# view-sonic/Cloud-Server

Measured on AMD Instinct MI355X. Metric: train_samples_per_s, higher is better.
Workload: dtype fp32; 1 GPU; model=reference sample CNN (API.md:306-332), 2,276,218 params, global_batch=50, per_gpu_batch=50, optimizer=AdagradOptimizer, parallelism=dp1, backend=hip, hip_graph=True, collectives=none, xgmi=single rank

## Files before the change

cloud_server_amd/csrc/kernels/dense_update.h:

```cpp
#pragma once
#include "common.h"
#include "optim_common.h"

namespace csa {

typedef float du_f32x4 __attribute__((ext_vector_type(4)));
typedef unsigned int du_u32x4 __attribute__((ext_vector_type(4)));

constexpr int DU_FT = 16;
constexpr int DU_SUB = 2;
constexpr int DU_MAXM = 64;
constexpr int DU_KS = DU_MAXM / 4;
constexpr int MAXC_DU = 128;
constexpr int DU_SLAB = 16;
constexpr int DU_PART = DU_MAXM * DU_FT;
constexpr size_t DU_LDS_MAX = 150 * 1024;

struct DUArgs {
  int M, K, N;
  const float* dY;
  float* W;
  float* bias;
  float* dX;
  const float* x_fwd;
  int act; float alpha;
  BNRef bn; int bn_on;
  const float* bn_tab;
  float* bwd_slab;
  int det;
  const float* Xw;
  int opt; float lr; const int64_t* step;
  float* s0w; float* s1w;
  float* s0b; float* s1b;
  float scale;
  float* gW; float* gb;
  int cs;
  float* part;
  unsigned* cnt;
  const float* hy;
  const float* hdl;
  float* hgw; float* hgb;
  const float* hrl; const int* hrc;
  float* ring_loss; int* ring_correct; int ring; float ldiv;
  int hact; float halpha;
  float* hw; float* hb; float* hs0w; float* hs1w; float* hs0b; float* hs1b;
};

constexpr int DU_HNC = 10;

constexpr int DU_MAXDEF = 4;
struct DUDeferred {
  DUArgs seg[DU_MAXDEF];
  int blocks[DU_MAXDEF];
  int n = 0;
  int head = -1;
};
extern thread_local DUDeferred g_du_def;

struct DUSegs {
  DUArgs seg[DU_MAXDEF];
  int start[DU_MAXDEF + 1];
  int nseg, head;
};
int du_take(DUSegs& out);
int du_flush_segs(const DUSegs& u, hipStream_t st);
}
extern "C" int csa_dense_update_flush(hipStream_t st);
namespace csa {


static __constant__ long long* g_du_dbg = nullptr;
#define DU_STAMP(i)                                                                          \
  do {                                                                                       \
    if (g_du_dbg && threadIdx.x == 0) g_du_dbg[bid * 16 + (i)] = (long long)__builtin_amdgcn_s_memrealtime(); \
  } while (0)

__host__ __device__ constexpr int du_nb(int waves) { return 32 * waves; }
constexpr int DU_FOLD_FS = 5, DU_FOLD_BLK = DU_FT * DU_FOLD_FS;
__host__ __device__ constexpr int du_upo_hw_floats() { return 64 * (8 + 10); }
__host__ __device__ inline size_t du_upo_lds_floats(int M) {
  const size_t m4 = (size_t)((M + 3) & ~3);
  const size_t tail = 1024 > du_upo_hw_floats() ? 1024 : du_upo_hw_floats();
  return 2 * m4 * 64 + tail;
}
__host__ __device__ inline size_t du_lds_floats(int M, int waves) {
  const size_t a = (size_t)M * (du_nb(waves) + 4), b = (size_t)waves * 4 * 4 * DU_FOLD_BLK;
  return (a > b ? a : b) + DU_MAXM * DU_FT + 6 * MAXC_DU + 4;
}

__device__ __forceinline__ du_u32x4 du_bits(float4 v) { du_u32x4 u; __builtin_memcpy(&u, &v, 16); return u; }
__device__ __forceinline__ float4 du_f4(du_u32x4 u) { float4 v; __builtin_memcpy(&v, &u, 16); return v; }

template <int NSLOT>
__device__ __forceinline__ void du_store_w(const DUArgs& a, const float4 (&wv)[DU_SUB], const float4 (&s0v)[DU_SUB],
                                           const float4 (&s1v)[DU_SUB], const long (&wofs)[DU_SUB],
                                           const bool (&sok)[DU_SUB], int i, int nf, bool bown, int bn0, float bw,
                                           float bs0, float bs1) {
  if (bown && (threadIdx.x & 63) == 0) {
    (a.gW ? a.gb : a.bias)[bn0] = bw;
    if (NSLOT >= 1) a.s0b[bn0] = bs0;
    if (NSLOT >= 2) a.s1b[bn0] = bs1;
  }
#pragma unroll
  for (int j = 0; j < DU_SUB; ++j) {
    if (!sok[j] || i >= nf) continue;
    *reinterpret_cast<float4*>((a.gW ? a.gW : a.W) + wofs[j]) = wv[j];
    if (NSLOT >= 1) *reinterpret_cast<float4*>(a.s0w + wofs[j]) = s0v[j];
    if (NSLOT >= 2) *reinterpret_cast<float4*>(a.s1w + wofs[j]) = s1v[j];
  }
}

constexpr int DU_HMAXR = 8;

struct DUHead {
  int hn0, nh;
  float hy[2];
  float dl[3];
};

template <int THREADS>
__device__ __forceinline__ void du_head_prefetch(const DUArgs& a, int grp, int groups, int cb, int nb, DUHead& h) {
  const int hper = (nb + groups - 1) / groups;
  h.hn0 = cb + grp * hper;
  h.nh = max(0, min(hper, cb + nb - h.hn0));
  const int t = threadIdx.x;
#pragma unroll
  for (int u = 0; u < 2; ++u) {
    const int e = t + u * THREADS, m = e / DU_HMAXR, r = e % DU_HMAXR;
    h.hy[u] = a.hy[(long)min(m, a.M - 1) * a.N + min(h.hn0 + min(r, max(h.nh - 1, 0)), a.N - 1)];
  }
  const int n10 = a.M * DU_HNC;
#pragma unroll
  for (int u = 0; u < 3; ++u) h.dl[u] = a.hdl[min(t + u * THREADS, n10 - 1)];
}

template <int THREADS>
__device__ __forceinline__ void du_head_finish(const DUArgs& a, DUHead& h, float* s_hw, bool last_block) {
  const int t = threadIdx.x, M = a.M;
  float* s_y = s_hw;
  float* s_d = s_hw + 64 * DU_HMAXR;
  pin(h.hy[0]); pin(h.hy[1]); pin(h.dl[0]); pin(h.dl[1]); pin(h.dl[2]);
  if (t < M * DU_HMAXR) s_y[t] = act_fwd(h.hy[0], a.hact, a.halpha);
  if (t + THREADS < M * DU_HMAXR) s_y[t + THREADS] = act_fwd(h.hy[1], a.hact, a.halpha);
#pragma unroll
  for (int u = 0; u < 3; ++u)
    if (t + u * THREADS < M * DU_HNC) s_d[t + u * THREADS] = h.dl[u];
  __syncthreads();
  const int outs = h.nh * DU_HNC;
  for (int o = t; o < outs; o += THREADS) {
    const int rr = o / DU_HNC, j = o - rr * DU_HNC, n = h.hn0 + rr;
    float v = 0.f;
    if (h.nh <= DU_HMAXR) {
      for (int m = 0; m < M; ++m) v = fmaf(s_y[m * DU_HMAXR + rr], s_d[m * DU_HNC + j], v);
    } else {
      for (int m = 0; m < M; ++m) v = fmaf(act_fwd(a.hy[(long)m * a.N + n], a.hact, a.halpha), s_d[m * DU_HNC + j], v);
    }
    if (a.hw) {
      const long k = (long)n * DU_HNC + j;
      float w = a.hw[k], z0 = a.hs0w ? a.hs0w[k] : 0.f, z1 = a.hs1w ? a.hs1w[k] : 0.f;
      opt_update(a.opt, opt_step_lr(a.opt, a.lr, a.step), w, v, z0, z1);
      a.hw[k] = w;
      if (a.hs0w) a.hs0w[k] = z0;
      if (a.hs1w) a.hs1w[k] = z1;
    } else {
      a.hgw[(long)n * DU_HNC + j] = v;
    }
  }
  if (last_block) {
    const int lane = t & 63, w = t >> 6;
    if (w == 0) {
      if (lane < DU_HNC) {
        float v = 0.f;
        for (int m = 0; m < M; ++m) v += s_d[m * DU_HNC + lane];
        if (a.hb) {
          float wb = a.hb[lane], z0 = a.hs0b ? a.hs0b[lane] : 0.f, z1 = a.hs1b ? a.hs1b[lane] : 0.f;
          opt_update(a.opt, opt_step_lr(a.opt, a.lr, a.step), wb, v, z0, z1);
          a.hb[lane] = wb;
          if (a.hs0b) a.hs0b[lane] = z0;
          if (a.hs1b) a.hs1b[lane] = z1;
        } else {
          a.hgb[lane] = v;
        }
      }
    } else if (w == 1) {
      float l = lane < M ? a.hrl[lane] : 0.f;
      float c = lane < M ? (float)a.hrc[lane] : 0.f;
      l = wave_sum(l);
      c = wave_sum(c);
      if (lane == 0) {
        const int pos = (int)((*a.step - 1) % a.ring);
        a.ring_loss[pos] = l / a.ldiv;
        a.ring_correct[pos] = (int)(c + 0.5f);
      }
    }
  }
}

template <int NSLOT, int WAVES, bool HEAD, bool DGO = false, bool UPO = false>
__device__ __forceinline__ void du_body(const DUArgs& a, const int bid, const int nblk, float* smem) {
  constexpr int THREADS = 64 * WAVES, NB = du_nb(WAVES), SN = NB + 4, HW = 16 * WAVES;
  const int M = a.M, K = a.K, N = a.N, cs = a.cs;
  static_assert(!UPO || WAVES == 4, "the update-only body is the 4-wave carried form");
  float* sdy = smem;
  float* s_bn = smem + du_lds_floats(M, WAVES) - 6 * MAXC_DU - 4;
  const int M4 = (M + 3) & ~3;
  float* sxw = UPO ? smem + 2 * M4 * 64 : s_bn - DU_MAXM * DU_FT;
  float* s_st = s_bn + 4 * MAXC_DU;
  int* s_flag = reinterpret_cast<int*>(s_st + 2 * MAXC_DU);
  const int tid = threadIdx.x, lane = tid & 63;
  const int wave = __builtin_amdgcn_readfirstlane(tid >> 6);
  const int i = lane & 15, q = lane >> 4;
  const int grp = bid / cs, cblk = bid - grp * cs;
  const int f0 = grp * DU_FT, nf = min(DU_FT, K - f0);
  const int cb = cblk * NB, nb = min(NB, N - cb);
  const int groups = nblk / cs;
  const bool dgrad = !UPO && a.dX != nullptr;
  const bool tf = dgrad && (a.act != ACT_NONE || a.bn_on);
  const bool tabs = a.bn_on && a.bn_tab;
  const int C = a.bn.C > 0 ? a.bn.C : 1;
  constexpr int nslot = NSLOT;
  DU_STAMP(0);
  float* s_hw;
  if constexpr (UPO) {
    s_hw = sxw;
  } else {
    __shared__ float s_hw_st[HEAD ? 64 * (DU_HMAXR + DU_HNC) : 1];
    s_hw = s_hw_st;
  }
  DUHead hd;

  float xw1[1024 / THREADS];
#pragma unroll
  for (int u = 0; u < 1024 / THREADS; ++u) {
    const int e = u * THREADS + tid;
    if (!DGO) xw1[u] = a.Xw[(long)min(e >> 4, M - 1) * K + f0 + min(e & 15, nf - 1)];
  }
  const float* tsrc = tabs ? a.bn_tab : a.Xw;
  float tv[512 / THREADS > 0 ? 512 / THREADS : 1];
  constexpr int NTV = UPO ? 0 : (512 / THREADS > 0 ? 512 / THREADS : 1);
#pragma unroll
  for (int u = 0; u < NTV; ++u) {
    const int e = u * THREADS + tid;
    tv[u] = tsrc[tabs && e < 4 * C ? e : 0];
  }
  const int n4 = N >> 2;
  int h4[DU_SUB];
#pragma unroll
  for (int j = 0; j < DU_SUB; ++j) h4[j] = max(min(nb - HW * j, HW), 0) >> 2;
  const float* b0 = nslot >= 1 ? a.s0w : a.W;
  const float* b1 = nslot >= 2 ? a.s1w : a.W;
  const int frow = f0 + min(i, nf - 1);
  float4 dyv[DU_SUB][4], wv[DU_SUB], s0v[DU_SUB], s1v[DU_SUB];
  long wofs[DU_SUB];
  bool sok[DU_SUB];
#pragma unroll
  for (int j = 0; j < DU_SUB; ++j) {
    if constexpr (UPO) {
      const int nch = M4 >> 2;
#pragma unroll
      for (int u = 0; u < DU_MAXM / 16; ++u) {
        const int c = min(wave + 4 * u, nch - 1);
        const int r = 4 * c + (lane >> 4), cq = ((lane & 15) - r) & 15;
        const float* src = a.dY + (long)min(r, M - 1) * N + cb + HW * j + 4 * cq;
        __builtin_amdgcn_global_load_lds(src, sdy + (j * M4 + 4 * c) * 64, 16, 0, 0);
      }
    } else {
#pragma unroll
    for (int u = 0; u < 4; ++u) {
      const int e = u * THREADS + tid;
      int row = 0, c4 = 0;
      if (h4[j] == HW / 4) { row = e / (HW / 4); c4 = e % (HW / 4); }
      else if (h4[j] > 0) { row = e / h4[j]; c4 = e - row * h4[j]; }
      dyv[j][u] = reinterpret_cast<const float4*>(a.dY)[min(row, M - 1) * n4 + (h4[j] > 0 ? (cb + HW * j) / 4 + c4 : 0)];
    }
    }
    const int lc = 16 * (wave + WAVES * j);
    sok[j] = lc < nb;
    wofs[j] = (long)frow * N + cb + min(lc, nb - 16) + 4 * q;
    wv[j] = *reinterpret_cast<const float4*>(a.W + wofs[j]);
    s0v[j] = s1v[j] = make_float4(0.f, 0.f, 0.f, 0.f);
    if (nslot >= 1) s0v[j] = *reinterpret_cast<const float4*>(b0 + wofs[j]);
    if (nslot >= 2) s1v[j] = *reinterpret_cast<const float4*>(b1 + wofs[j]);
  }
  const int bper = (nb + groups - 1) / groups;
  const int bn0 = cb + grp * bper + wave;
  const bool bown = !DGO && (a.bias || a.gW) && wave < bper && grp * bper + wave < nb;
  const int bnc = bown ? bn0 : 0;
  float bw = (a.bias ? a.bias : a.dY)[bnc];
  float bs0 = (nslot >= 1 && a.bias ? a.s0b : a.dY)[bnc];
  float bs1 = (nslot >= 2 && a.bias ? a.s1b : a.dY)[bnc];
  const int em = tid >> 2, fq = 4 * (tid & 3);
  const bool eitem = tid < 256;
  const float* xsrc = tf && a.x_fwd ? a.x_fwd : a.Xw;
  float4 xf = make_float4(0.f, 0.f, 0.f, 0.f);
  if (!UPO) xf = *reinterpret_cast<const float4*>(xsrc + (long)min(em, M - 1) * K + f0 + min(fq, nf - 4));
  if (HEAD) du_head_prefetch<THREADS>(a, grp, groups, cb, nb, hd);

  const float lr = opt_step_lr(a.opt, a.lr, a.step);
  du_f32x4 dacc[4];
#pragma unroll
  for (int t = 0; t < 4; ++t) dacc[t] = du_f32x4{0.f, 0.f, 0.f, 0.f};
  float xb[DU_KS];
#pragma unroll
  for (int j = 0; j < DU_SUB; ++j) {
    if (j == 0) {
#pragma unroll
      for (int u = 0; u < 1024 / THREADS; ++u) {
        if (DGO) break;
        const int e = u * THREADS + tid;
        pin(xw1[u]);
        sxw[e] = ((e >> 4) < M && (e & 15) < nf) ? xw1[u] : 0.f;
      }
#pragma unroll
      for (int u = 0; u < NTV; ++u) {
        const int e = u * THREADS + tid;
        pin(tv[u]);
        if (tabs && e < 4 * C) s_bn[(e / C) * MAXC_DU + e % C] = tv[u];
      }
    }
    if constexpr (!UPO) {
#pragma unroll
    for (int u = 0; u < 4; ++u) pin(dyv[j][u]);
#pragma unroll
    for (int u = 0; u < 4; ++u) {
      const int e = u * THREADS + tid;
      if (h4[j] > 0 && e < M * h4[j]) {
        const int row = h4[j] == HW / 4 ? e / (HW / 4) : e / h4[j];
        const int c4 = e - row * h4[j];
        *reinterpret_cast<float4*>(sdy + row * SN + HW * j + 4 * c4) = dyv[j][u];
      }
    }
    }
    if (j == 0 && a.bn_on && dgrad && !tabs)
      bn_reduce_to_lds(a.bn, s_bn, s_bn + MAXC_DU, s_bn + 2 * MAXC_DU, s_bn + 3 * MAXC_DU, s_st);
    __syncthreads();
    if (UPO && j == 1) DU_STAMP(4);
    if (j == 0) {
      DU_STAMP(1);
#pragma unroll
      for (int s = 0; s < DU_KS; ++s) xb[s] = DGO ? 0.f : sxw[(4 * s + q) * DU_FT + i];
    }
    pin(wv[j]); pin(s0v[j]); pin(s1v[j]);
    if (j == 0) DU_STAMP(2);
    if (UPO && j == 1) DU_STAMP(5);
    if (!sok[j]) continue;
    const int n0 = 16 * (wave + WAVES * j);
    const float wk[4] = {wv[j].x, wv[j].y, wv[j].z, wv[j].w};
    if (dgrad) {
#pragma unroll
      for (int t = 0; t < 4; ++t) {
        if (16 * t >= M) break;
        const float4 d4 = *reinterpret_cast<const float4*>(sdy + min(16 * t + i, M - 1) * SN + n0 + 4 * q);
        const float ak[4] = {d4.x, d4.y, d4.z, d4.w};
#pragma unroll
        for (int k = 0; k < 4; ++k) dacc[t] = __builtin_amdgcn_mfma_f32_16x16x4f32(ak[k], i < nf ? wk[k] : 0.f, dacc[t], 0, 0, 0);
      }
    }
    if (DGO) continue;
    du_f32x4 g0 = du_f32x4{0.f, 0.f, 0.f, 0.f}, g1 = g0;
    const float* col = sdy + n0 + i;
    float av[DU_KS];
    if constexpr (UPO) {
      const float* hb = sdy + j * M4 * 64;
      const int lc = 16 * wave + i;
#pragma unroll
      for (int s = 0; s < DU_KS; ++s) {
        const int r = min(4 * s + q, M - 1);
        av[s] = hb[r * 64 + ((((lc >> 2) + r) & 15) << 2) + (lc & 3)];
      }
    } else {
#pragma unroll
      for (int s = 0; s < DU_KS; ++s) av[s] = col[min(4 * s + q, M - 1) * SN];
    }
#pragma unroll
    for (int s = 0; s < DU_KS; s += 2) {
      g0 = __builtin_amdgcn_mfma_f32_16x16x4f32(av[s], xb[s], g0, 0, 0, 0);
      g1 = __builtin_amdgcn_mfma_f32_16x16x4f32(av[s + 1], xb[s + 1], g1, 0, 0, 0);
    }
    float w[4] = {wv[j].x, wv[j].y, wv[j].z, wv[j].w};
    float s0[4] = {s0v[j].x, s0v[j].y, s0v[j].z, s0v[j].w};
    float s1[4] = {s1v[j].x, s1v[j].y, s1v[j].z, s1v[j].w};
#pragma unroll
    for (int r = 0; r < 4; ++r) {
      if (a.gW) w[r] = (g0[r] + g1[r]) * a.scale;
      else opt_update(a.opt, lr, w[r], (g0[r] + g1[r]) * a.scale, s0[r], s1[r]);
    }
    wv[j] = make_float4(w[0], w[1], w[2], w[3]);
    s0v[j] = make_float4(s0[0], s0[1], s0[2], s0[3]);
    s1v[j] = make_float4(s1[0], s1[1], s1[2], s1[3]);
    if (UPO && j == 0) DU_STAMP(7);
    if (UPO && j == 1) DU_STAMP(8);
  }
  pin(bw); pin(bs0); pin(bs1); pin(xf);
  if (bown) {
    for (int u = wave; u < bper; u += WAVES) {
      const int lcol = grp * bper + u;
      if (lcol >= nb) break;
      const int n = cb + lcol;
      float v;
      if constexpr (UPO) {
        const int lh = lcol & 63;
        v = lane < M ? sdy[((lcol >> 6) * M4 + lane) * 64 + ((((lh >> 2) + lane) & 15) << 2) + (lh & 3)] : 0.f;
      } else {
        v = lane < M ? sdy[lane * SN + lcol] : 0.f;
      }
      v = wave_sum(v);
      if (lane == 0) {
        if (u == wave) {
          if (a.gW) bw = v * a.scale;
          else opt_update(a.opt, lr, bw, v * a.scale, bs0, bs1);
        } else {
          float cw = 0.f, c0 = 0.f, c1 = 0.f;
          if (!a.gW) {
            cw = a.bias[n];
            if (nslot >= 1) c0 = a.s0b[n];
            if (nslot >= 2) c1 = a.s1b[n];
          }
          if (a.gW) cw = v * a.scale;
          else opt_update(a.opt, lr, cw, v * a.scale, c0, c1);
          (a.gW ? a.gb : a.bias)[n] = cw;
          if (nslot >= 1) a.s0b[n] = c0;
          if (nslot >= 2) a.s1b[n] = c1;
        }
      }
    }
  }
  DU_STAMP(3);
  if (HEAD) du_head_finish<THREADS>(a, hd, s_hw, bid == nblk - 1);
  if (!dgrad) {
    if (!DGO) du_store_w<NSLOT>(a, wv, s0v, s1v, wofs, sok, i, nf, bown, bn0, bw, bs0, bs1);
    DU_STAMP(6);
    return;
  }

  __syncthreads();
  float* fold = sdy;
#pragma unroll
  for (int t = 0; t < 4; ++t) {
    if (16 * t >= M) break;
    float* dst = fold + ((wave * 4 + t) * 4 + q) * DU_FOLD_BLK + DU_FOLD_FS * i;
#pragma unroll
    for (int r = 0; r < 4; ++r) dst[r] = dacc[t][r];
  }
  __syncthreads();
  DU_STAMP(4);
  float4 g4 = make_float4(0.f, 0.f, 0.f, 0.f);
  if (eitem && em < M) {
    const int t = em >> 4, qq = (em >> 2) & 3, r = em & 3;
    const float* src = fold + (t * 4 + qq) * DU_FOLD_BLK + DU_FOLD_FS * fq + r;
#pragma unroll
    for (int w = 0; w < WAVES; ++w) {
      const float* p = src + w * 4 * 4 * DU_FOLD_BLK;
      g4.x += p[0]; g4.y += p[DU_FOLD_FS]; g4.z += p[2 * DU_FOLD_FS]; g4.w += p[3 * DU_FOLD_FS];
    }
  }
  if (cs > 1) {
    const __amdgpu_buffer_rsrc_t prs = __builtin_amdgcn_make_buffer_rsrc(
        a.part, 0, (int)((size_t)nblk * DU_PART * sizeof(float)), 0x00020000);
    if (eitem && em < M)
      __builtin_amdgcn_raw_buffer_store_b128(du_bits(g4), prs, (int)(((size_t)bid * DU_PART + em * DU_FT + fq) * 4), 0, 16);
    asm volatile("s_waitcnt vmcnt(0)" ::: "memory");
    __syncthreads();
    if (tid == 0) {
      const unsigned old = __hip_atomic_fetch_add(a.cnt + grp, 1u, __ATOMIC_RELAXED, __HIP_MEMORY_SCOPE_AGENT);
      const int last = old == (unsigned)(cs - 1);
      if (last) __hip_atomic_store(a.cnt + grp, 0u, __ATOMIC_RELAXED, __HIP_MEMORY_SCOPE_AGENT);
      *s_flag = last;
    }
    __syncthreads();
    if (!DGO) du_store_w<NSLOT>(a, wv, s0v, s1v, wofs, sok, i, nf, bown, bn0, bw, bs0, bs1);
    if (!*s_flag) return;
    __builtin_amdgcn_fence(__ATOMIC_ACQUIRE, "wavefront");
    g4 = make_float4(0.f, 0.f, 0.f, 0.f);
    if (eitem && em < M) {
      float4 v[8];
      for (int c0 = 0; c0 < cs; c0 += 8) {
#pragma unroll
        for (int u = 0; u < 8; ++u)
          v[u] = du_f4(__builtin_amdgcn_raw_buffer_load_b128(
              prs, (int)((((size_t)grp * cs + min(c0 + u, cs - 1)) * DU_PART + em * DU_FT + fq) * 4), 0, 16));
#pragma unroll
        for (int u = 0; u < 8; ++u)
          if (c0 + u < cs) { g4.x += v[u].x; g4.y += v[u].y; g4.z += v[u].z; g4.w += v[u].w; }
      }
    }
  } else {
    if (!DGO) du_store_w<NSLOT>(a, wv, s0v, s1v, wofs, sok, i, nf, bown, bn0, bw, bs0, bs1);
  }
  float v1[4] = {0.f, 0.f, 0.f, 0.f}, v2[4] = {0.f, 0.f, 0.f, 0.f};
  if (eitem && em < M && fq < nf) {
    float g[4] = {g4.x, g4.y, g4.z, g4.w};
    const float x[4] = {xf.x, xf.y, xf.z, xf.w};
    if (tf) {
      int ch = (f0 + fq) % C;
#pragma unroll
      for (int r = 0; r < 4; ++r, ch = (ch + 1 == C) ? 0 : ch + 1) {
        const float z = a.bn_on ? x[r] * s_bn[2 * MAXC_DU + ch] + s_bn[3 * MAXC_DU + ch] : x[r];
        const float y = act_fwd(z, a.act, a.alpha);
        g[r] = act_bwd(g[r], z, y, a.act, a.alpha);
        v1[r] = g[r];
        v2[r] = a.bn_on ? g[r] * (x[r] - s_bn[ch]) * s_bn[MAXC_DU + ch] : 0.f;
      }
    }
    out_store4(a.dX + (long)em * K + f0 + fq, make_float4(g[0], g[1], g[2], g[3]));
  }
  DU_STAMP(5);
  if (a.bn_on && a.bwd_slab) {
#pragma unroll
    for (int r = 0; r < 4; ++r) {
#pragma unroll
      for (int o = 4; o < 64; o <<= 1) {
        v1[r] += __shfl_xor(v1[r], o, 64);
        v2[r] += __shfl_xor(v2[r], o, 64);
      }
    }
    float* sred = sxw;
    if (eitem && lane < 4) {
#pragma unroll
      for (int r = 0; r < 4; ++r) {
        sred[wave * 32 + 4 * lane + r] = v1[r];
        sred[wave * 32 + 16 + 4 * lane + r] = v2[r];
      }
    }
    __syncthreads();
    if (a.det) {
      if (tid < 2 * C) {
        const int st = tid / C, c = tid - st * C;
        float acc = 0.f;
        for (int ff = 0; ff < nf; ++ff)
          if ((f0 + ff) % C == c) {
            const int e = 16 * st + ff;
            acc += sred[e] + sred[32 + e] + sred[64 + e] + sred[96 + e];
          }
        a.bwd_slab[(size_t)grp * 2 * C + tid] = acc;
      }
    } else if (tid < 32 && (tid & 15) < nf) {
      const float acc = sred[tid] + sred[32 + tid] + sred[64 + tid] + sred[96 + tid];
      const int st = tid >> 4, c = (f0 + (tid & 15)) % C;
      atomicAdd(a.bwd_slab + (size_t)(grp % DU_SLAB) * 2 * C + st * C + c, acc);
    }
  }
  DU_STAMP(6);
}

template <int NSLOT, bool HEADOK>
__device__ __forceinline__ void du_segs_body(const DUSegs& u, int e, float* smem) {
  int s = 0;
#pragma unroll
  for (int k = 1; k < DU_MAXDEF; ++k) s += (k < u.nseg && e >= u.start[k]) ? 1 : 0;
  const DUArgs& d = u.seg[s];
  const int lb = e - u.start[s], nb = u.start[s + 1] - u.start[s];
  if (HEADOK && s == u.head) du_body<NSLOT, 4, true, false, true>(d, lb, nb, smem);
  else du_body<NSLOT, 4, false, false, true>(d, lb, nb, smem);
}

}
```

cloud_server_amd/csrc/kernels/dense_update.hip:

```cpp
#include "dense_update.h"
#include <cstdlib>

namespace csa {

template <int NSLOT, int WAVES, bool HEAD, bool DGO = false>
__global__ __launch_bounds__(64 * WAVES) void dense_bwd_update_kernel(DUArgs a) {
  extern __shared__ __attribute__((aligned(16))) float smem[];
  du_body<NSLOT, WAVES, HEAD, DGO>(a, (int)blockIdx.x, (int)gridDim.x, smem);
}

thread_local DUDeferred g_du_def{};

}


using namespace csa;

static thread_local float* g_du_grad_w = nullptr;
static thread_local float* g_du_grad_b = nullptr;

CSA_NT_SETTER(csa_nt_out_du)

CSA_API int csa_du_debug(long long* p) {
  return (int)hipMemcpyToSymbol(HIP_SYMBOL(g_du_dbg), &p, sizeof(p));
}

CSA_API int csa_dense_bwd_update_ok(int M, int K, int N, int bn_C) {
  if (M < 1 || M > DU_MAXM || K < 4 || K % 4 || N < 16 || N % 16) return 0;
  if (bn_C > MAXC_DU) return 0;
  if (N > 512 && N % 128) return 0;
  return du_lds_floats(M, 16) * sizeof(float) <= DU_LDS_MAX ? 1 : 0;
}

CSA_API int csa_dense_bwd_update_slabs(int K) {
  const int groups = (K + DU_FT - 1) / DU_FT;
  return g_csa_det || groups < DU_SLAB ? groups : DU_SLAB;
}

static int du_cs(int K, int N) {
  const int groups = (K + DU_FT - 1) / DU_FT;
  static const int wide_env = [] { const char* e = getenv("CSA_DU_WIDE"); return e ? (e[0] == '0' ? 0 : 1) : -1; }();
  const bool narrow = wide_env == 0 || g_csa_shared || (g_csa_packed && wide_env != 1);
  const int minb = narrow ? (1 << 30) : 128;
  if (N <= 512 && groups >= minb) return 1;
  return (N + 127) / 128;
}

CSA_API int csa_dense_bwd_update_ws(int K, int N, long long* ws) {
  const long long groups = (K + DU_FT - 1) / DU_FT, cs = du_cs(K, N);
  ws[0] = cs > 1 ? groups * cs * DU_PART : 0;
  ws[1] = cs > 1 ? groups : 0;
  return (int)cs;
}

template <int NSLOT, int WAVES, bool HEAD>
static void du_launch3(const DUArgs& a, int blocks, hipStream_t st) {
  static const bool attr = hipFuncSetAttribute((const void*)dense_bwd_update_kernel<NSLOT, WAVES, HEAD>,
                                               hipFuncAttributeMaxDynamicSharedMemorySize, (int)DU_LDS_MAX) == hipSuccess;
  (void)attr;
  hipLaunchKernelGGL((dense_bwd_update_kernel<NSLOT, WAVES, HEAD>), dim3((unsigned)blocks), dim3(64 * WAVES),
                     du_lds_floats(a.M, WAVES) * sizeof(float), st, a);
}

template <int WAVES>
static void du_launch3_dgo(const DUArgs& a, int blocks, hipStream_t st) {
  static const bool attr = hipFuncSetAttribute((const void*)dense_bwd_update_kernel<0, WAVES, false, true>,
                                               hipFuncAttributeMaxDynamicSharedMemorySize, (int)DU_LDS_MAX) == hipSuccess;
  (void)attr;
  hipLaunchKernelGGL((dense_bwd_update_kernel<0, WAVES, false, true>), dim3((unsigned)blocks), dim3(64 * WAVES),
                     du_lds_floats(a.M, WAVES) * sizeof(float), st, a);
}

template <int NSLOT, int WAVES>
static void du_launch(const DUArgs& a, int blocks, hipStream_t st) {
  if (a.hy) du_launch3<NSLOT, WAVES, true>(a, blocks, st);
  else du_launch3<NSLOT, WAVES, false>(a, blocks, st);
}

CSA_API int csa_dense_bwd_update_head(const float* dY, float* W, float* bias, float* dX, int M, int K, int N,
                                      const float* x_fwd, int act, float alpha, const float* bn_slab, int bn_nslab,
                                      int bn_C, float bn_count, float bn_eps, const float* bn_scale,
                                      const float* bn_offset, float* bwd_slab, const float* Xw, int opt, float lr,
                                      const int64_t* step, float* s0w, float* s1w, float* s0b, float* s1b,
                                      float scale, const float* bn_tab, float* part, unsigned* cnt,
                                      const float* hy, const float* hdl, float* hgw, float* hgb, const float* hrl,
                                      const int* hrc, float* ring_loss, int* ring_correct, int ring, float ldiv,
                                      int hact, float halpha, hipStream_t st);

CSA_API int csa_dense_bwd_update(const float* dY, float* W, float* bias, float* dX, int M, int K, int N,
                                 const float* x_fwd, int act, float alpha, const float* bn_slab, int bn_nslab,
                                 int bn_C, float bn_count, float bn_eps, const float* bn_scale,
                                 const float* bn_offset, float* bwd_slab, const float* Xw, int opt, float lr,
                                 const int64_t* step, float* s0w, float* s1w, float* s0b, float* s1b,
                                 float scale, const float* bn_tab, float* part, unsigned* cnt, hipStream_t st) {
  return csa_dense_bwd_update_head(dY, W, bias, dX, M, K, N, x_fwd, act, alpha, bn_slab, bn_nslab, bn_C, bn_count,
                                   bn_eps, bn_scale, bn_offset, bwd_slab, Xw, opt, lr, step, s0w, s1w, s0b, s1b,
                                   scale, bn_tab, part, cnt, nullptr, nullptr, nullptr, nullptr, nullptr, nullptr,
                                   nullptr, nullptr, 1, 1.f, 0, 0.f, st);
}

CSA_API int csa_dense_bwd_grad_head(const float* dY, const float* W, float* dX, int M, int K, int N,
                                    const float* x_fwd, int act, float alpha, const float* bn_slab, int bn_nslab,
                                    int bn_C, float bn_count, float bn_eps, const float* bn_scale,
                                    const float* bn_offset, float* bwd_slab, const float* Xw, float scale,
                                    const float* bn_tab, float* part, unsigned* cnt, float* gW, float* gb,
                                    const float* hy, const float* hdl, float* hgw, float* hgb, const float* hrl,
                                    const int* hrc, float* ring_loss, int* ring_correct, int ring, float ldiv,
                                    int hact, float halpha, const int64_t* step, hipStream_t st);

CSA_API int csa_dense_bwd_update_head(const float* dY, float* W, float* bias, float* dX, int M, int K, int N,
                                 const float* x_fwd, int act, float alpha, const float* bn_slab, int bn_nslab,
                                 int bn_C, float bn_count, float bn_eps, const float* bn_scale,
                                 const float* bn_offset, float* bwd_slab, const float* Xw, int opt, float lr,
                                 const int64_t* step, float* s0w, float* s1w, float* s0b, float* s1b,
                                 float scale, const float* bn_tab, float* part, unsigned* cnt,
                                      const float* hy, const float* hdl, float* hgw, float* hgb, const float* hrl,
                                      const int* hrc, float* ring_loss, int* ring_correct, int ring, float ldiv,
                                      int hact, float halpha, hipStream_t st) {
  if (!csa_dense_bwd_update_ok(M, K, N, bn_slab ? bn_C : 0)) return -1;
  if (hy && (!hdl || !hgw || !hgb || !hrl || !hrc || !ring_loss || !ring_correct || ring < 1 || !step)) return -2;
  if (!Xw || !W || !dY) return -2;
  DUArgs a{};
  a.M = M; a.K = K; a.N = N; a.dY = dY; a.W = W; a.bias = bias; a.dX = dX; a.x_fwd = x_fwd;
  a.act = act; a.alpha = alpha;
  a.bn = BNRef{bn_slab, bn_nslab, bn_slab ? bn_C : 1, bn_count, bn_eps, bn_scale, bn_offset};
  a.bn_on = bn_slab != nullptr; a.bn_tab = bn_slab ? bn_tab : nullptr;
  a.bwd_slab = bwd_slab; a.Xw = Xw; a.det = g_csa_det;
  a.opt = opt; a.lr = lr; a.step = step; a.s0w = s0w; a.s1w = s1w; a.s0b = s0b; a.s1b = s1b; a.scale = scale;
  const int groups = (K + DU_FT - 1) / DU_FT;
  a.cs = du_cs(K, N);
  a.part = part; a.cnt = cnt;
  a.hy = hy; a.hdl = hdl; a.hgw = hgw; a.hgb = hgb; a.hrl = hrl; a.hrc = hrc;
  a.ring_loss = ring_loss; a.ring_correct = ring_correct; a.ring = ring; a.ldiv = ldiv;
  a.hact = hact; a.halpha = halpha;
  a.gW = g_du_grad_w; a.gb = g_du_grad_b;
  if (a.cs > 1 && dX && (!part || !cnt)) return -2;
  const int blocks = groups * a.cs;
  const int ns = a.gW ? 0 : opt_nslots(opt);
  if (a.cs == 1) {
    if (ns == 0) du_launch<0, 16>(a, blocks, st);
    else if (ns == 1) du_launch<1, 16>(a, blocks, st);
    else du_launch<2, 16>(a, blocks, st);
  } else {
    if (ns == 0) du_launch<0, 4>(a, blocks, st);
    else if (ns == 1) du_launch<1, 4>(a, blocks, st);
    else du_launch<2, 4>(a, blocks, st);
  }
  return (int)hipGetLastError();
}

CSA_API int csa_dense_bwd_grad_head(const float* dY, const float* W, float* dX, int M, int K, int N,
                                    const float* x_fwd, int act, float alpha, const float* bn_slab, int bn_nslab,
                                    int bn_C, float bn_count, float bn_eps, const float* bn_scale,
                                    const float* bn_offset, float* bwd_slab, const float* Xw, float scale,
                                    const float* bn_tab, float* part, unsigned* cnt, float* gW, float* gb,
                                    const float* hy, const float* hdl, float* hgw, float* hgb, const float* hrl,
                                    const int* hrc, float* ring_loss, int* ring_correct, int ring, float ldiv,
                                    int hact, float halpha, const int64_t* step, hipStream_t st) {
  if (!gW || !gb) return -2;
  g_du_grad_w = gW;
  g_du_grad_b = gb;
  const int rc = csa_dense_bwd_update_head(dY, const_cast<float*>(W), nullptr, dX, M, K, N, x_fwd, act, alpha,
                                           bn_slab, bn_nslab, bn_C, bn_count, bn_eps, bn_scale, bn_offset,
                                           bwd_slab, Xw, OPT_SGD, 0.f, step, nullptr, nullptr, nullptr, nullptr,
                                           scale, bn_tab, part, cnt, hy, hdl, hgw, hgb, hrl, hrc, ring_loss,
                                           ring_correct, ring, ldiv, hact, halpha, st);
  g_du_grad_w = g_du_grad_b = nullptr;
  return rc;
}


CSA_API int csa_dense_bwd_dgrad(const float* dY, const float* W, float* dX, int M, int K, int N,
                                const float* x_fwd, int act, float alpha, const float* bn_slab, int bn_nslab,
                                int bn_C, float bn_count, float bn_eps, const float* bn_scale,
                                const float* bn_offset, float* bwd_slab, const float* bn_tab, float* part,
                                unsigned* cnt, hipStream_t st) {
  if (!csa_dense_bwd_update_ok(M, K, N, bn_slab ? bn_C : 0) || !dX || !dY || !W) return -1;
  DUArgs a{};
  a.M = M; a.K = K; a.N = N; a.dY = dY; a.W = const_cast<float*>(W); a.dX = dX; a.x_fwd = x_fwd;
  a.act = act; a.alpha = alpha;
  a.bn = BNRef{bn_slab, bn_nslab, bn_slab ? bn_C : 1, bn_count, bn_eps, bn_scale, bn_offset};
  a.bn_on = bn_slab != nullptr; a.bn_tab = bn_slab ? bn_tab : nullptr;
  a.bwd_slab = bwd_slab; a.Xw = x_fwd ? x_fwd : dX; a.det = g_csa_det; a.scale = 1.f;
  const int groups = (K + DU_FT - 1) / DU_FT;
  a.cs = du_cs(K, N);
  a.part = part; a.cnt = cnt;
  if (a.cs > 1 && (!part || !cnt)) return -2;
  const int blocks = groups * a.cs;
  if (a.cs == 1) du_launch3_dgo<16>(a, blocks, st);
  else du_launch3_dgo<4>(a, blocks, st);
  return (int)hipGetLastError();
}

CSA_API int csa_dense_update_defer(const float* dY, float* W, float* bias, int M, int K, int N, const float* Xw,
                                   int opt, float lr, const int64_t* step, float* s0w, float* s1w, float* s0b,
                                   float* s1b, float scale, const float* hy, const float* hdl, float* hgw,
                                   float* hgb, const float* hrl, const int* hrc, float* ring_loss,
                                   int* ring_correct, int ring, float ldiv, int hact, float halpha) {
  if (!csa_dense_bwd_update_ok(M, K, N, 0) || N % 128 || !Xw || !W || !dY || !step) return -1;
  if (g_du_def.n >= DU_MAXDEF) return -3;
  if (hy && (g_du_def.head >= 0 || !hdl || !hgw || !hgb || !hrl || !hrc || !ring_loss || !ring_correct || ring < 1))
    return -2;
  if (g_du_def.n > 0 && opt_nslots(g_du_def.seg[0].opt) != opt_nslots(opt)) return -4;
  DUArgs a{};
  a.M = M; a.K = K; a.N = N; a.dY = dY; a.W = W; a.bias = bias; a.dX = nullptr; a.x_fwd = nullptr;
  a.bn = BNRef{nullptr, 0, 1, 1.f, 0.f, nullptr, nullptr};
  a.Xw = Xw; a.det = g_csa_det;
  a.opt = opt; a.lr = lr; a.step = step; a.s0w = s0w; a.s1w = s1w; a.s0b = s0b; a.s1b = s1b; a.scale = scale;
  a.cs = N / 128;
  a.hy = hy; a.hdl = hdl; a.hgw = hgw; a.hgb = hgb; a.hrl = hrl; a.hrc = hrc;
  a.ring_loss = ring_loss; a.ring_correct = ring_correct; a.ring = ring; a.ldiv = ldiv;
  a.hact = hact; a.halpha = halpha;
  if (g_du_def.n == 0) g_du_def.head = -1;
  if (hy) g_du_def.head = g_du_def.n;
  g_du_def.blocks[g_du_def.n] = ((K + DU_FT - 1) / DU_FT) * a.cs;
  g_du_def.seg[g_du_def.n++] = a;
  return g_du_def.n;
}

CSA_API int csa_dense_update_pending() { return g_du_def.n; }

CSA_API int csa_dense_update_grad_mode(float* gW, float* gb) {
  if (g_du_def.n < 1 || !gW || !gb) return -1;
  DUArgs& a = g_du_def.seg[g_du_def.n - 1];
  if (opt_nslots(a.opt) != 0) return -2;
  a.gW = gW; a.gb = gb;
  return 0;
}

CSA_API int csa_dense_update_head_params(float* hw, float* hb, float* hs0w, float* hs1w, float* hs0b, float* hs1b) {
  if (g_du_def.head < 0 || !hw || !hb) return -1;
  DUArgs& a = g_du_def.seg[g_du_def.head];
  const int ns = opt_nslots(a.opt);
  if ((ns >= 1 && (!hs0w || !hs0b)) || (ns >= 2 && (!hs1w || !hs1b))) return -2;
  a.hw = hw; a.hb = hb; a.hs0w = hs0w; a.hs1w = hs1w; a.hs0b = hs0b; a.hs1b = hs1b;
  return 0;
}

namespace csa {
int du_take(DUSegs& out) {
  out = DUSegs{};
  out.head = g_du_def.head;
  out.nseg = g_du_def.n;
  for (int s = 0; s < DU_MAXDEF; ++s) {
    if (s < out.nseg) out.seg[s] = g_du_def.seg[s];
    out.start[s + 1] = out.start[s] + (s < out.nseg ? g_du_def.blocks[s] : 0);
  }
  g_du_def.n = 0;
  g_du_def.head = -1;
  return out.nseg;
}
}

namespace csa {
int du_flush_segs(const DUSegs& u, hipStream_t st) {
  for (int s = 0; s < u.nseg; ++s) {
    const DUArgs& a = u.seg[s];
    const int ns = opt_nslots(a.opt), blocks = u.start[s + 1] - u.start[s];
    const bool head = s == u.head;
    if (ns == 0) head ? du_launch3<0, 4, true>(a, blocks, st) : du_launch3<0, 4, false>(a, blocks, st);
    else if (ns == 1) head ? du_launch3<1, 4, true>(a, blocks, st) : du_launch3<1, 4, false>(a, blocks, st);
    else head ? du_launch3<2, 4, true>(a, blocks, st) : du_launch3<2, 4, false>(a, blocks, st);
  }
  return (int)hipGetLastError();
}
}

CSA_API int csa_dense_update_flush(hipStream_t st) {
  DUSegs u;
  return du_take(u) > 0 ? du_flush_segs(u, st) : 0;
}

CSA_API void csa_dense_update_clear() { g_du_def.n = 0; g_du_def.head = -1; }

CSA_API int csa_dense_update_flush_last(hipStream_t st) {
  const int n = g_du_def.n;
  if (n < 1) return 0;
  DUSegs u{};
  u.nseg = 1;
  u.head = g_du_def.head == n - 1 ? 0 : -1;
  u.seg[0] = g_du_def.seg[n - 1];
  u.start[0] = 0;
  for (int s2 = 1; s2 <= DU_MAXDEF; ++s2) u.start[s2] = g_du_def.blocks[n - 1];
  g_du_def.n = n - 1;
  if (g_du_def.head == n - 1) g_du_def.head = -1;
  return du_flush_segs(u, st);
}
```

Before: 710,000 samples/s.

## Add dedicated dgrad-only kernel for single-chunk dense backward

Adds a standalone 1024-thread dense_dgrad_kernel for the cs==1 dgrad path. Each wave loads up to two 16-wide N chunks of dY and W, computes partial dX tiles with fp32 MFMA, and reduces the 16 wave partials through LDS before applying the activation/BN backward and BN stat accumulation. It replaces the generic du_body template instantiation, which carries extra update and LDS staging machinery. A vmcnt wait is also inserted in the update-only path of du_body. The new kernel handles only N up to 512 (two chunks per wave across 16 waves), which risks incorrect results for larger N if the existing guards do not exclude them.

```diff
diff --git a/cloud_server_amd/csrc/kernels/dense_update.h b/cloud_server_amd/csrc/kernels/dense_update.h
--- a/cloud_server_amd/csrc/kernels/dense_update.h
+++ b/cloud_server_amd/csrc/kernels/dense_update.h
@@ -318,6 +318,7 @@
         if (tabs && e < 4 * C) s_bn[(e / C) * MAXC_DU + e % C] = tv[u];
       }
     }
+    if (UPO && j == 0) asm volatile("s_waitcnt vmcnt(0)" ::: "memory");
     if constexpr (!UPO) {
 #pragma unroll
     for (int u = 0; u < 4; ++u) pin(dyv[j][u]);
diff --git a/cloud_server_amd/csrc/kernels/dense_update.hip b/cloud_server_amd/csrc/kernels/dense_update.hip
--- a/cloud_server_amd/csrc/kernels/dense_update.hip
+++ b/cloud_server_amd/csrc/kernels/dense_update.hip
@@ -7,6 +7,135 @@
 __global__ __launch_bounds__(64 * WAVES) void dense_bwd_update_kernel(DUArgs a) {
   extern __shared__ __attribute__((aligned(16))) float smem[];
   du_body<NSLOT, WAVES, HEAD, DGO>(a, (int)blockIdx.x, (int)gridDim.x, smem);
+}
+
+constexpr int DG_CH = 2;
+constexpr int DG_PART = 16 * 4 * 4 * 64;
+constexpr size_t DG_LDS = (DG_PART + 6 * MAXC_DU + 16 * 32) * sizeof(float);
+
+__global__ __launch_bounds__(1024) void dense_dgrad_kernel(DUArgs a) {
+  extern __shared__ __attribute__((aligned(16))) float smem[];
+  float* s_bn = smem + DG_PART;
+  float* s_red = s_bn + 6 * MAXC_DU;
+  const int M = a.M, K = a.K, N = a.N;
+  const int bid = (int)blockIdx.x, tid = threadIdx.x, lane = tid & 63;
+  const int wave = __builtin_amdgcn_readfirstlane(tid >> 6);
+  const int i = lane & 15, q = lane >> 4;
+  const int f0 = bid * DU_FT, nf = min(DU_FT, K - f0);
+  const bool tf = a.act != ACT_NONE || a.bn_on;
+  const bool tabs = a.bn_on && a.bn_tab;
+  const int C = a.bn.C > 0 ? a.bn.C : 1;
+  const int nch = N >> 4;
+  const int et = wave & 3, er = wave >> 2;
+  DU_STAMP(0);
+
+  const unsigned wo = (unsigned)(min(i, nf - 1) * N + 4 * q) * 4u;
+  unsigned dyo[4];
+#pragma unroll
+  for (int t = 0; t < 4; ++t) dyo[t] = (unsigned)(min(16 * t + i, M - 1) * N + 4 * q) * 4u;
+  const char* dyb = reinterpret_cast<const char*>(a.dY);
+  const char* wb = reinterpret_cast<const char*>(a.W + (long)f0 * N);
+  float4 dyv[DG_CH][4], wv[DG_CH];
+#pragma unroll
+  for (int u = 0; u < DG_CH; ++u) {
+    const int c = min(wave + 16 * u, nch - 1);
+    wv[u] = *reinterpret_cast<const float4*>(wb + 64 * c + wo);
+#pragma unroll
+    for (int t = 0; t < 4; ++t) dyv[u][t] = *reinterpret_cast<const float4*>(dyb + 64 * c + dyo[t]);
+    __builtin_amdgcn_sched_barrier(0);
+  }
+  const int ch = (f0 + i) % C;
+  const int em = 16 * et + 4 * q + er;
+  const float* tsrc = tabs ? a.bn_tab : a.dY;
+  float xv = (a.x_fwd ? a.x_fwd : a.dX)[(long)min(em, M - 1) * K + f0 + min(i, nf - 1)];
+  float tb[4];
+#pragma unroll
+  for (int k = 0; k < 4; ++k) tb[k] = tsrc[tabs ? k * C + ch : 0];
+  if (a.bn_on && !tabs) {
+    bn_reduce_to_lds(a.bn, s_bn, s_bn + MAXC_DU, s_bn + 2 * MAXC_DU, s_bn + 3 * MAXC_DU, s_bn + 4 * MAXC_DU);
+    __syncthreads();
+#pragma unroll
+    for (int k = 0; k < 4; ++k) tb[k] = s_bn[k * MAXC_DU + ch];
+  }
+
+  du_f32x4 acc[4];
+#pragma unroll
+  for (int t = 0; t < 4; ++t) acc[t] = du_f32x4{0.f, 0.f, 0.f, 0.f};
+#pragma unroll
+  for (int u = 0; u < DG_CH; ++u) {
+    pin(wv[u]);
+#pragma unroll
+    for (int t = 0; t < 4; ++t) pin(dyv[u][t]);
+    if (u == 0) { DU_STAMP(1); DU_STAMP(2); }
+    if (wave + 16 * u >= nch) continue;
+    const float wk[4] = {wv[u].x, wv[u].y, wv[u].z, wv[u].w};
+#pragma unroll
+    for (int t = 0; t < 4; ++t) {
+      if (16 * t >= M) break;
+      const float ak[4] = {dyv[u][t].x, dyv[u][t].y, dyv[u][t].z, dyv[u][t].w};
+#pragma unroll
+      for (int k = 0; k < 4; ++k) acc[t] = __builtin_amdgcn_mfma_f32_16x16x4f32(ak[k], wk[k], acc[t], 0, 0, 0);
+    }
+  }
+  DU_STAMP(3);
+  pin(xv);
+#pragma unroll
+  for (int k = 0; k < 4; ++k) pin(tb[k]);
+
+#pragma unroll
+  for (int t = 0; t < 4; ++t) {
+    if (16 * t >= M) break;
+#pragma unroll
+    for (int r = 0; r < 4; ++r) smem[((wave * 4 + t) * 4 + r) * 64 + lane] = acc[t][r];
+  }
+  __syncthreads();
+  const bool stats = a.bn_on && a.bwd_slab;
+  const bool live = 16 * et < M;
+  float v1 = 0.f, v2 = 0.f;
+  if (live) {
+    float g = 0.f;
+    const float* src = smem + (et * 4 + er) * 64 + lane;
+#pragma unroll
+    for (int w = 0; w < 16; ++w) g += src[w * 16 * 64];
+    DU_STAMP(4);
+    float d2 = 0.f;
+    if (tf) {
+      const float z = a.bn_on ? xv * tb[2] + tb[3] : xv;
+      const float y = act_fwd(z, a.act, a.alpha);
+      g = act_bwd(g, z, y, a.act, a.alpha);
+      d2 = a.bn_on ? g * (xv - tb[0]) * tb[1] : 0.f;
+    }
+    if (em < M && i < nf) {
+      out_store(a.dX + (long)em * K + f0 + i, g);
+      v1 = g;
+      v2 = d2;
+    }
+    DU_STAMP(5);
+  }
+  if (stats) {
+    v1 += __shfl_xor(v1, 16, 64); v2 += __shfl_xor(v2, 16, 64);
+    v1 += __shfl_xor(v1, 32, 64); v2 += __shfl_xor(v2, 32, 64);
+    if (q == 0) { s_red[wave * 32 + i] = v1; s_red[wave * 32 + 16 + i] = v2; }
+    __syncthreads();
+    if (a.det) {
+      if (tid < 2 * C) {
+        const int st = tid >= C ? 1 : 0, c = tid - st * C;
+        float sum = 0.f;
+        int cc = f0 % C;
+        for (int ff = 0; ff < nf; ++ff, cc = (cc + 1 == C) ? 0 : cc + 1)
+          if (cc == c)
+            for (int w = 0; w < 16; ++w) sum += s_red[w * 32 + 16 * st + ff];
+        a.bwd_slab[(size_t)bid * 2 * C + tid] = sum;
+      }
+    } else if (tid < 32 && (tid & 15) < nf) {
+      float sum = 0.f;
+#pragma unroll
+      for (int w = 0; w < 16; ++w) sum += s_red[w * 32 + tid];
+      const int st = tid >> 4, c = (f0 + (tid & 15)) % C;
+      atomicAdd(a.bwd_slab + (size_t)(bid % DU_SLAB) * 2 * C + st * C + c, sum);
+    }
+  }
+  DU_STAMP(6);
 }
 
 thread_local DUDeferred g_du_def{};
@@ -62,13 +191,12 @@
                      du_lds_floats(a.M, WAVES) * sizeof(float), st, a);
 }
 
-template <int WAVES>
-static void du_launch3_dgo(const DUArgs& a, int blocks, hipStream_t st) {
-  static const bool attr = hipFuncSetAttribute((const void*)dense_bwd_update_kernel<0, WAVES, false, true>,
+static void du_launch3_dgo4(const DUArgs& a, int blocks, hipStream_t st) {
+  static const bool attr = hipFuncSetAttribute((const void*)dense_bwd_update_kernel<0, 4, false, true>,
                                                hipFuncAttributeMaxDynamicSharedMemorySize, (int)DU_LDS_MAX) == hipSuccess;
   (void)attr;
-  hipLaunchKernelGGL((dense_bwd_update_kernel<0, WAVES, false, true>), dim3((unsigned)blocks), dim3(64 * WAVES),
-                     du_lds_floats(a.M, WAVES) * sizeof(float), st, a);
+  hipLaunchKernelGGL((dense_bwd_update_kernel<0, 4, false, true>), dim3((unsigned)blocks), dim3(64 * 4),
+                     du_lds_floats(a.M, 4) * sizeof(float), st, a);
 }
 
 template <int NSLOT, int WAVES>
@@ -187,8 +315,12 @@
   a.part = part; a.cnt = cnt;
   if (a.cs > 1 && (!part || !cnt)) return -2;
   const int blocks = groups * a.cs;
-  if (a.cs == 1) du_launch3_dgo<16>(a, blocks, st);
-  else du_launch3_dgo<4>(a, blocks, st);
+  if (a.cs == 1) {
+    static const bool attr = hipFuncSetAttribute((const void*)dense_dgrad_kernel,
+                                                 hipFuncAttributeMaxDynamicSharedMemorySize, (int)DG_LDS) == hipSuccess;
+    (void)attr;
+    hipLaunchKernelGGL(dense_dgrad_kernel, dim3((unsigned)blocks), dim3(1024), DG_LDS, st, a);
+  } else du_launch3_dgo4(a, blocks, st);
   return (int)hipGetLastError();
 }
 
```

Result: faster. 745,600 samples/s, median of 6 (+5.0%).
